# hasindu2008/squigulator

Hardware: AMD Instinct MI355X
Metric: simulated raw samples/sec (higher is better)
Workload: dtype f32+f64

## Files before the change

### squigulator_amd/csrc/h_common.h

```cpp
#pragma once

#if defined(SQG_DEV)
#define SQG_DEV_ENV(name) getenv(name)
#else
#define SQG_DEV_ENV(name) (static_cast<const char*>(nullptr))
#endif
static inline int dev_env_int(const char* v, int dflt) { return v ? atoi(v) : dflt; }

#ifndef SQG_SOURCE_HASH
#define SQG_SOURCE_HASH "unstamped"
#endif
extern "C" const char sqg_source_hash_marker[] = "SQG_SOURCE_HASH=" SQG_SOURCE_HASH ";";
#if defined(SQG_DEV)
static const char kBuildInfo[] = "source_hash=" SQG_SOURCE_HASH ";dev=1";
#else
static const char kBuildInfo[] = "source_hash=" SQG_SOURCE_HASH ";dev=0";
#endif
extern "C" const char* sqg_build_info(void) { return kBuildInfo; }

#include "h_cpus.h"

static uint32_t lcg_pow(uint32_t base, unsigned long long e) {
    uint32_t r = 1, b = base;
    while (e) { if (e & 1) r = lcg_mul(r, b); b = lcg_mul(b, b); e >>= 1; }
// ... 59 lines not shown
    DevBuf<long long> d_span; std::vector<long long> h_span;
    DevBuf<ChunkView> d_view;
    const void* span_of = nullptr; unsigned long long span_run = 0;
    void release() { *this = ChunkScratch(); }
};

struct SiteScratch {
    DevBuf<int> d_count; std::vector<int> h_count;
    DevBuf<long long> d_off; std::vector<long long> h_off;
    DevBuf<SiteRec> d_rec;
    DevBuf<uint8_t> d_skip;
    const void* plan_of = nullptr; unsigned long long plan_run = 0; int plan_key[3] = {0, 0, 0};
    void release() { *this = SiteScratch(); }
};

struct EventScratch {
    DevBuf<long long> d_start;
    DevBuf<int> d_read;
    void release() { *this = EventScratch(); }
};

struct PileupScratch {
    DevBuf<uint32_t> d_kmer;
    DevBuf<uint8_t> d_seg;
    DevBuf<PileRead> d_pr; std::vector<PileRead> h_pr;
    DevBuf<unsigned long long> d_stat;
    void release() { *this = PileupScratch(); }
};

struct DetectScratch {
    DevBuf<int> d_count; std::vector<int> h_count;
    DevBuf<long long> d_off; std::vector<long long> h_off;
    DevBuf<long long> d_start;
    DevBuf<int> d_read;
    void release() { *this = DetectScratch(); }
};

struct AlignScratch {
    DevBuf<long long> d_off;
    DevBuf<int16_t> d_level;
    DevBuf<ulonglong2> d_mask; DevBuf<int> d_lo;
    DevBuf<int> d_end;
    void release() { *this = AlignScratch(); }
};

struct sqg_ctx {
    HostPool pool_threads;
    struct DrawAhead* draw_ahead = nullptr;
    sqg_cfg_t cfg;
    int k = 0, num_kmer = 0, T = 0, wlo = 0, whi = 0, nw = 0;
    hipStream_t stream = nullptr;
    uint32_t* d_rows = nullptr;
    float2* d_model = nullptr;
    uint32_t* d_pow = nullptr;
    std::vector<uint32_t> h_pow;
    uint32_t jump2(unsigned long long n) const {
        if (n >> 32) return lcg_pow(lcg_mul(LCG_A, LCG_A), n);
        uint32_t r = h_pow[2 * POW_N + (size_t)(n & (POW_N - 1))];
        const uint32_t hi = (uint32_t)(n >> 10) & (POW_N - 1), hi2 = (uint32_t)(n >> 20);
        if (hi) r = lcg_mul(r, h_pow[3 * POW_N + hi]);
        if (hi2) r = lcg_mul(r, h_pow[4 * POW_N + hi2]);
        return r;
    }
    unsigned int* d_err = nullptr;
    unsigned long long fix_tickets = 0;
    unsigned long long scan_tickets = 0;
    struct Slot {
        int16_t* d_sig = nullptr; size_t sig_cap = 0;
        long long* d_sigoff = nullptr; size_t reads_cap = 0;
        FixEntry* d_fix = nullptr; size_t fix_cap = 0;
        unsigned int* d_fix_count = nullptr;
        FixEntry* d_fix_sh = nullptr; size_t fix_sh_cap = 0;
        unsigned int fix_sh_per = 0;
        unsigned int* d_fix_sh_count = nullptr;
        uint2* d_evrec = nullptr; size_t evrec_cap = 0;
        int* d_slow = nullptr; size_t slow_cap = 0;
        ItemDesc* d_items = nullptr; size_t items_cap = 0;
        uint32_t* d_part = nullptr; size_t part_cap = 0;
        uint32_t* d_lbase = nullptr; size_t lbase_cap = 0;
        int* d_tile_link = nullptr; size_t tile_link_cap = 0;
        uint32_t* d_part_state = nullptr; size_t part_state_cap = 0;
        hipEvent_t cal_a = nullptr, cal_b = nullptr; bool cal_pending = false; long long cal_events = 0; int cal_tries = 0; float cal_ps = 0.f;
        uint2* cal_prev = nullptr; float cal_prev_ps = 0.f;
        unsigned long long gen = 0;
        hipEvent_t done = nullptr;
        hipEvent_t sampled = nullptr;
    } slot[2];
    struct CountSet {
        uint16_t* d_dwell = nullptr; size_t dwell_cap = 0;
        uint32_t* d_tile_so = nullptr; size_t tile_cap = 0;
        unsigned long long* d_seglen = nullptr; size_t seglen_cap = 0;
        size_t seglen_dirty = 0;
        unsigned long long gen = 0;
    } cset[3];
    int num_cu = 256;
    std::deque<sqg_batch*> staged_q;
    hipStream_t fix_stream = nullptr;
    unsigned long long* d_scan_part = nullptr; size_t scan_part_cap = 0;
    uint32_t* d_link_rows = nullptr; size_t link_rows_cap = 0;
    uint32_t* d_pcnt[2] = {nullptr, nullptr}; size_t pcnt_cap[2] = {0, 0};
    uint32_t* d_slice = nullptr; size_t slice_cap = 0;
    uint32_t* d_phist = nullptr; size_t phist_cap = 0;
    double row_bound = 0;
    bool range_mode = false;
    uint32_t* d_xcounts = nullptr; size_t xcounts_cap = 0;
    struct Recycled { uint8_t* d_block; size_t block_bytes; long long* h_sigoff; long long* h_sigoff_dev; size_t h_n; hipEvent_t ev[8];
// ... 266 lines not shown
```

### squigulator_amd/csrc/h_context.h

```cpp
#pragma once

extern "C" const char* sqg_strerror(int code) {
    switch (code) {
    case SQG_OK: return "ok";
    case SQG_EINVAL: return "invalid argument or unsupported configuration";
    case SQG_ENOMEM: return "out of memory";
    case SQG_EDEVICE: return "HIP runtime error";
    case SQG_ESEQUENCE: return "batches must be run in staging order";
    case SQG_ENODEVICE: return "no usable HIP device";
    case SQG_EOVERFLOW: return "read too long (>= UINT32_MAX samples) or dwell > 65535";
    case SQG_EIO: return "file I/O error";
    default: return "unknown error";
    }
}

extern "C" const char* sqg_last_error(const sqg_ctx_t* ctx) { return ctx ? ctx->err.c_str() : ""; }

extern "C" int sqg_device_count(void) {
    int n = 0;
    if (hipGetDeviceCount(&n) != hipSuccess) return SQG_ENODEVICE;
    return n;
}

extern "C" int32_t sqg_worker_of(int32_t i, int32_t n_rec, int32_t T) {
    if (T <= 1 || n_rec <= 0) return 0;
    const int32_t step = (n_rec + T - 1) / T;
    return i / step;
}

extern "C" void sqg_destroy(sqg_ctx_t* ctx) {
    if (!ctx) return;
    if (ctx->b5_reader_drain) ctx->b5_reader_drain(ctx->b5_reader, true);
    (void)hipSetDevice(ctx->cfg.device);
    if (ctx->b5_stream) { (void)hipStreamSynchronize(ctx->b5_stream); (void)hipStreamDestroy(ctx->b5_stream); ctx->b5_stream = nullptr; }
    if (ctx->stream) (void)hipStreamSynchronize(ctx->stream);
    if (ctx->fix_stream) (void)hipStreamSynchronize(ctx->fix_stream);
    delete ctx->draw_ahead; ctx->draw_ahead = nullptr;
    (void)hipFree(ctx->d_pcnt[0]); (void)hipFree(ctx->d_pcnt[1]); (void)hipFree(ctx->d_slice); (void)hipFree(ctx->d_phist);
    (void)hipFree(ctx->d_rows); (void)hipFree(ctx->d_link_rows); (void)hipFree(ctx->d_scan_part); (void)hipFree(ctx->d_xcounts); (void)hipFree(ctx->d_model); (void)hipFree(ctx->d_samp_scratch); (void)hipFree(ctx->d_pow); (void)hipFree(ctx->d_err); (void)hipFree(ctx->d_mid_done); if (ctx->h_samp) (void)hipHostFree(ctx->h_samp);
    for (auto& Q : ctx->cset) { (void)hipFree(Q.d_dwell); (void)hipFree(Q.d_tile_so); (void)hipFree(Q.d_seglen); }
    for (auto& S : ctx->slot) {
        (void)hipFree(S.d_sig); (void)hipFree(S.d_sigoff);
        (void)hipFree(S.d_fix); (void)hipFree(S.d_fix_count); (void)hipFree(S.d_fix_sh); (void)hipFree(S.d_fix_sh_count);
        (void)hipFree(S.d_evrec); (void)hipFree(S.d_slow);
        (void)hipFree(S.d_items); (void)hipFree(S.d_part_state); (void)hipFree(S.d_part); (void)hipFree(S.d_lbase); (void)hipFree(S.d_tile_link);
        (void)hipFree(S.cal_prev);
        if (S.cal_a) (void)hipEventDestroy(S.cal_a);
        if (S.cal_b) (void)hipEventDestroy(S.cal_b);
        if (S.done) (void)hipEventDestroy(S.done);
        if (S.sampled) (void)hipEventDestroy(S.sampled);
    }
    (void)hipFree(ctx->d_svb); (void)hipFree(ctx->d_svb_size); (void)hipFree(ctx->d_svb_off);
    (void)hipFree(ctx->d_b5meta); (void)hipFree(ctx->d_b5out); (void)hipFree(ctx->d_b5tab); (void)hipFree(ctx->d_b5size); for (auto* q : ctx->h_b5out) if (q) (void)hipHostFree(q); if (ctx->h_b5meta) (void)hipHostFree(ctx->h_b5meta);
    ctx->chunk.release();
    ctx->site.release();
    ctx->event.release();
    ctx->pileup.release();
    ctx->detect.release();
    ctx->align.release();
    (void)hipFree(ctx->d_genome); (void)hipFree(ctx->d_contig_off); (void)hipFree(ctx->d_cum); (void)hipFree(ctx->d_nprefix);
    (void)hipFree(ctx->d_trans_csum); (void)hipFree(ctx->d_trans_idx); (void)hipFree(ctx->d_samp);
    (void)hipFree(ctx->d_meth); (void)hipFree(ctx->d_meth_has); (void)hipFree(ctx->d_meth_st);
    if (ctx->stage_stream) { (void)hipStreamSynchronize(ctx->stage_stream); (void)hipStreamDestroy(ctx->stage_stream); }
    for (auto& r : ctx->pool) { (void)hipFree(r.d_block); (void)hipHostFree(r.h_sigoff); (void)hipHostFree(r.h_meta); for (auto& e : r.ev) if (e) (void)hipEventDestroy(e); if (r.ev_staged) (void)hipEventDestroy(r.ev_staged); }
    ctx->pool.clear();
    if (ctx->fix_stream) (void)hipStreamDestroy(ctx->fix_stream);
    if (ctx->stream) (void)hipStreamDestroy(ctx->stream);
    delete ctx;
}

extern "C" int sqg_create(const sqg_cfg_t* cfg, sqg_ctx_t** out) {
    if (!cfg || !out) return SQG_EINVAL;
    *out = nullptr;
    if (cfg->abi_version != SQG_ABI_VERSION) return SQG_EINVAL;
    if (cfg->kmer_size < 1 || cfg->kmer_size > 9 || !cfg->model) return SQG_EINVAL;
    if (cfg->num_workers < 1 || cfg->worker_lo < 0 || cfg->worker_hi > cfg->num_workers || cfg->worker_lo >= cfg->worker_hi) return SQG_EINVAL;
    if (!(cfg->profile.range != 0.0) || !(cfg->profile.dwell_mean >= 1.0)) return SQG_EINVAL;
    if (cfg->profile.dwell_mean + 8.0 * std::fabs(cfg->profile.dwell_std) > 60000.0) return SQG_EINVAL;
    if (cfg->mode != SQG_MODE_EXACT && cfg->mode != SQG_MODE_CERTIFIED) return SQG_EINVAL;
    long long nk = 1LL << (2 * cfg->kmer_size);
    if (cfg->flags & SQG_METH) { nk = 1; for (uint32_t i = 0; i < cfg->kmer_size; i++) nk *= 5; }
    const double span = std::fabs((double)cfg->seed) + (double)cfg->num_workers * (double)(nk + 10);
    if (span > 9.0e10) return SQG_EINVAL;

    int ndev = 0;
    if (hipGetDeviceCount(&ndev) != hipSuccess || ndev <= 0) return SQG_ENODEVICE;
    if (cfg->device < 0 || cfg->device >= ndev) return SQG_EINVAL;

    sqg_ctx* c = new (std::nothrow) sqg_ctx();
    if (!c) return SQG_ENOMEM;
    c->cfg = *cfg;
    c->cfg.model = nullptr;
// ... 42 lines not shown
    CHK(hipMemset(c->d_err, 0, sizeof(unsigned int)));
    CHK(hipStreamCreateWithFlags(&c->stage_stream, hipStreamNonBlocking));
    {
        int prio_lo = 0, prio_hi = 0;
        CHK(hipDeviceGetStreamPriorityRange(&prio_lo, &prio_hi));
        CHK(hipStreamCreateWithPriority(&c->fix_stream, hipStreamNonBlocking, prio_lo));
    }
    for (auto& S : c->slot) {
        CHK(hipMalloc(&S.d_fix_count, (4 + FIX_SHARDS) * sizeof(unsigned int)));
        CHK(hipMemset(S.d_fix_count, 0, (4 + FIX_SHARDS) * sizeof(unsigned int)));
        if (cfg->mode == SQG_MODE_CERTIFIED && c->use_kmer_streams) {
            CHK(hipMalloc(&S.d_fix_sh_count, (size_t)FIX_SHARDS * FIX_SHARD_STRIDE * sizeof(unsigned int)));
            CHK(hipMemset(S.d_fix_sh_count, 0, (size_t)FIX_SHARDS * FIX_SHARD_STRIDE * sizeof(unsigned int)));
        }
        CHK(hipEventCreateWithFlags(&S.done, hipEventDisableTiming));
        CHK(hipEventCreateWithFlags(&S.sampled, hipEventDisableTiming));
        CHK(hipEventRecord(S.done, c->stream));
    }
    if (c->use_kmer_streams && !SQG_DEV_ENV("SQG_PART_CLAIMS") && !(cfg->flags & SQG_ORDER_FREE)) {
        hipDeviceProp_t prop;
        CHK(hipGetDeviceProperties(&prop, cfg->device));
        const bool listed = strncmp(prop.gcnArchName, "gfx950", 6) == 0;
        if (!listed) fprintf(stderr, "[sqg] %s is not on the list of architectures verified for lane-ordered LDS atomics: extended probe\n", prop.gcnArchName);
        unsigned int* d_bad = nullptr;
        CHK(hipMalloc(&d_bad, sizeof(unsigned int)));
        CHK(hipMemset(d_bad, 0, sizeof(unsigned int)));
        hipLaunchKernelGGL(k_lds_order_check, dim3(1024), dim3(64), 0, c->stream, listed ? 4 : 64, d_bad);
        CHK(hipGetLastError());
        unsigned int bad = 1;
        CHK(hipMemcpyAsync(&bad, d_bad, sizeof bad, hipMemcpyDeviceToHost, c->stream));
        CHK(hipStreamSynchronize(c->stream));
        (void)hipFree(d_bad);
        c->lds_ordered = bad == 0;
        if (!c->lds_ordered) fprintf(stderr, "[sqg] LDS atomics are not served in lane order on this device (%u mismatches): the claim protocol hands the k-mer streams out\n", bad);
    }
    if (cfg->mode == SQG_MODE_CERTIFIED) {
        unsigned int* d_max = nullptr;
        CHK(hipMalloc(&d_max, sizeof(unsigned int)));
        CHK(hipMemset(d_max, 0, sizeof(unsigned int)));
        hipLaunchKernelGGL(k_certify, dim3(256 * 16), dim3(256), 0, c->stream, d_max);
        CHK(hipGetLastError());
        unsigned int bits = 0;
        CHK(hipMemcpyAsync(&bits, d_max, sizeof bits, hipMemcpyDeviceToHost, c->stream));
        CHK(hipStreamSynchronize(c->stream));
        (void)hipFree(d_max);
        float m; memcpy(&m, &bits, sizeof m);
        c->delta_x_measured = m;
        if (!(m < 1.0e-4f)) { fprintf(stderr, "[sqg] certification sweep failed: max error %g\n", (double)m); return fail(SQG_EDEVICE); }
        c->delta_x = m * 1.25f + 1.0e-7f;
        if (getenv("SQG_VERBOSE")) fprintf(stderr, "[sqg] certified fp32 deviate: max |x_fp32 - x_fp64| over all states = %.3e, bound used %.3e\n", (double)m, (double)c->delta_x);
        if (const char* ov = SQG_DEV_ENV("SQG_TEST_DELTA_X")) { c->delta_x = (float)atof(ov); c->force_fix = true; }
        const double kd = cfg->profile.digitisation / cfg->profile.range;
        double lo = 1e300, hi = -1e300, eps_max = 0;
        for (long long j = 0; j < nk; j++) {
            const double mkd = (double)hm[(size_t)j].x * kd;
            const float sdk = (float)((double)hm[(size_t)j].y * kd);
            const float asdk = std::fabs(sdk);
            lo = std::min(lo, mkd - 7.0 * asdk); hi = std::max(hi, mkd + 7.0 * asdk);
            const float eps = c->delta_x * asdk + 5.9604645e-8f * ((float)std::fabs(mkd) + 21.0f * asdk + 3.0f) + 2.0e-7f;
            eps_max = std::max(eps_max, (double)eps);
        }
        c->amp_floor = lo; c->amp_ceil = hi;
        c->thr_all = std::nextafterf((float)(0.5 - eps_max * 1.000001), 0.0f);
    }
    {
        const sqg_profile_t& q = cfg->profile;
        const double a = std::floor(q.dwell_mean + 6.5556 * std::fabs(q.dwell_std) + 0.5);
        const double z = std::floor(std::fabs(q.dwell_mean - 6.5556 * std::fabs(q.dwell_std)) + 0.5) + 1.0;
        c->dwell_hi = c->use_dwell_stream ? std::max(std::max(a, z), 1.0) + 1.0 : (double)(int)q.dwell_mean;
        const double mu = std::fabs(q.dwell_mean) + 0.5, sg = c->use_dwell_stream ? std::fabs(q.dwell_std) : 0.0;
        c->lean_epl = 1;
        for (int epl = LEAN_EPL_MAX; epl >= 1; epl >>= 1) {
            const double nev = 64.0 * epl;
            if (nev * mu + 6.0 * std::sqrt(nev) * sg <= 0.97 * LEAN_MAX_SAMPLES) { c->lean_epl = epl; break; }
        }
    }

    if (c->use_kmer_streams) {
        const long long total = (long long)c->nw * nk;
        CHK(hipMalloc(&c->d_rows, (size_t)total * sizeof(uint32_t)));
        if (c->num_kmer <= 4096) {
            const int blocks = (int)((total + 255) / 256);
            hipLaunchKernelGGL(k_init_rows, dim3(blocks), dim3(256), 0, c->stream, c->d_rows, (int)nk, (long long)cfg->seed, c->wlo, total);
            CHK(hipGetLastError());
        } else {
            const char* turns_env = SQG_DEV_ENV("SQG_TEST_ROW_TURNS");
            const int turns = turns_env ? std::min(3, std::max(0, atoi(turns_env))) : 0;
            CHK(hipMemsetD32Async((hipDeviceptr_t)c->d_rows, (int)((unsigned)turns * LCG_ORD2), (size_t)total, c->stream));
            c->row_bound = (double)turns * (double)LCG_ORD2 + (turns == 3 ? (double)LCG_ORD2 : 0.0);
        }
    }
    c->time_c.resize((size_t)c->nw); c->off_x.resize((size_t)c->nw); c->med_x.resize((size_t)c->nw);
    for (int w = 0; w < c->nw; w++) {
        const long long s = (long long)cfg->seed + (long long)(w + c->wlo) * (nk + 10);
        c->time_c[(size_t)w] = canon(s + 2);
        c->off_x[(size_t)w] = s + 4;
        c->med_x[(size_t)w] = s + 5;
    }
    CHK(hipStreamSynchronize(c->stream));
#undef CHK
    *out = c;
    return SQG_OK;
}
```

### squigulator_amd/csrc/h_run.h

```cpp
#pragma once

static void count_params(sqg_ctx* c, const sqg_batch* b, sqg_ctx::CountSet& Q, const int n_part, uint32_t* d_pcnt, SigParams& P) {
    const sqg_profile_t& p = c->cfg.profile;
    P.reads = b->d_reads; P.chain_off = b->d_chain_off; P.chain_reads = b->d_chain_reads; P.chain_order = b->d_chain_order; P.bases = b->d_bases;
    P.dwell = c->use_dwell_stream ? Q.d_dwell : nullptr; P.dwell_out = Q.d_dwell; P.seglen_out = Q.d_seglen; P.seglen = Q.d_seglen; P.tile_so = Q.d_tile_so;
    P.dmean = p.dwell_mean; P.dstd = p.dwell_std; P.pw = c->d_pow; P.err = b->d_err; P.delta_x = c->delta_x;
    P.k = c->k; P.num_kmer = c->num_kmer; P.const_sps = (int)p.dwell_mean;
    P.dwell_unbounded = c->dwell_hi > 65535.0 ? 1 : 0;
    P.dwell_pack = c->dwell_hi < 1024.0 ? 1 : 0;
    P.pieces = b->d_pieces; P.piece_total = b->d_piece_total;
    P.pcnt = d_pcnt; P.n_part = n_part; P.n_links = b->n_chains;
}

struct RunStep { const char* name; std::function<int()> go; };
typedef std::vector<RunStep> RunPlan;

struct Run {
    sqg_ctx* c; sqg_batch* b; int phase; const uint32_t* before; const uint32_t* after;
    sqg_ctx::Slot* S; sqg_ctx::Slot* other; sqg_ctx::CountSet* Q;
    int n = 0, n_part = 0, dw = 0;
    bool certified = false, direct = false, fold = false, untimed = false, wave_links = false;
    size_t n_pairs = 0, n_rows = 0;
    unsigned scan_wgs = 0, pgrid = 0;
    uint32_t *d_pcnt = nullptr, *slice_lo = nullptr, *slice_hi = nullptr, *pfirst = nullptr, *pstart = nullptr, *ptotal = nullptr;
// ... 56 lines not shown
        !c->range_mode && !c->staged_q.empty() && !SQG_DEV_ENV("SQG_NO_PRECOUNT")) {
        sqg_batch* cand = c->staged_q.front();
        if (cand->seq > b->seq && cand->staged && !cand->ran && !cand->begun && !cand->precounted && cand->part && cand->pieces && cand->one == b->one &&
            cand->n > 0 && cand->n_chains > 0) {
            sqg_ctx::CountSet& NQ = c->cset[(b->run_idx + 1) % 3];
            bool ok = grow_cset(c, NQ, cand) == SQG_OK;
            const int nx = (int)((b->run_idx + 1) & 1);
            if (ok && !cand->one) ok = ensure(c, (void**)&c->d_pcnt[nx], &c->pcnt_cap[nx], (size_t)2 * cand->n_chains * (size_t)R.n_part, sizeof(uint32_t)) == SQG_OK;
            if (ok && cand->one) ok = ensure(c, (void**)&other.d_part, &other.part_cap, (size_t)cand->n_events + PART_SLACK, sizeof(uint32_t)) == SQG_OK;
            if (ok) R.pre_nb = cand;
            else c->err.clear();
        }
    }
    if (phase != 2 && b->split && !b->part && (rc = ensure(c, (void**)&c->d_link_rows, &c->link_rows_cap, (size_t)b->n_chains * (size_t)c->num_kmer, sizeof(uint32_t)))) return rc;
    if (phase != 2 && b->part) {
        if ((rc = ensure(c, (void**)&c->d_pcnt[b->run_idx & 1], &c->pcnt_cap[b->run_idx & 1], (size_t)2 * b->n_chains * (size_t)R.n_part, sizeof(uint32_t)))) return rc;
        if ((rc = ensure(c, (void**)&c->d_slice, &c->slice_cap, (size_t)2 * (size_t)b->max_slices + (size_t)3 * R.n_pairs + 1, sizeof(uint32_t)))) return rc;
        if ((rc = ensure(c, (void**)&c->d_phist, &c->phist_cap, (size_t)b->max_slices * (size_t)PART_SUB, sizeof(uint32_t)))) return rc;
    }
    if (phase == 1 && (rc = ensure(c, (void**)&c->d_xcounts, &c->xcounts_cap, R.n_rows, sizeof(uint32_t)))) return rc;
    if (n > 0 && phase != 1) {
        const size_t cap0 = c->scan_part_cap;
        if ((rc = ensure(c, (void**)&c->d_scan_part, &c->scan_part_cap, (size_t)2 * R.scan_wgs, sizeof(unsigned long long)))) return rc;
        if (c->scan_part_cap != cap0)
            HIPCHK(c, hipMemsetAsync(c->d_scan_part, 0, c->scan_part_cap * sizeof(unsigned long long), c->stream));
    }
    return SQG_OK;
}

static void run_params(Run& R) {
    sqg_ctx* c = R.c; sqg_batch* b = R.b; const int phase = R.phase, n = R.n;
    sqg_ctx::Slot& S = *R.S; sqg_ctx::CountSet& Q = *R.Q;
    const sqg_profile_t& p = c->cfg.profile;
    R.direct = c->num_kmer <= 4096;
    R.dw = c->use_dwell_stream ? (R.certified && c->dwell_hi < 1.0e6 ? 1 : 2) : 0;
    R.wave_links = b->pieces;
    const int n_part = R.n_part;
    R.d_pcnt = c->d_pcnt[b->run_idx & 1];
    R.pgrid = (unsigned)b->max_slices;
    R.slice_lo = c->d_slice;
    R.slice_hi = R.slice_lo ? R.slice_lo + (size_t)b->max_slices : nullptr;
    R.pfirst = R.slice_hi ? R.slice_hi + (size_t)b->max_slices : nullptr;
    R.pstart = R.pfirst ? R.pfirst + R.n_pairs + 1 : nullptr;
    R.ptotal = R.pstart ? R.pstart + R.n_pairs : nullptr;
    SigParams& P = R.P;
    memset(&P, 0, sizeof P);
    P.link_rows = (b->split && !b->part) ? c->d_link_rows : nullptr;
    P.part = S.d_part; P.part_state = b->part ? S.d_part_state : nullptr;
    P.poff = b->one ? b->d_link_slot : R.d_pcnt ? R.d_pcnt + (size_t)b->n_chains * n_part : nullptr;
    P.link_q = b->d_link_q;
    P.one = b->one ? 1 : 0;
    count_params(c, b, Q, n_part, R.d_pcnt, P);
    P.pstart = R.pstart;
    P.sig_off = S.d_sigoff; P.model = c->d_model; P.rows = c->d_rows;
    P.seed_base = canon((long long)c->cfg.seed + (long long)c->wlo * ((long long)c->num_kmer + 10)); P.seed_step = canon((long long)c->num_kmer + 10);
    P.dig = p.digitisation; P.range = p.range; P.kd = p.digitisation / p.range;
    P.thr_all = c->thr_all;
    P.meth = (c->cfg.flags & SQG_METH) ? 1 : 0; P.num_kmer_pad = n_part * PART_SUB;
    P.meth_top = 1; for (int i = 1; i < c->k; i++) P.meth_top *= 5u;
    P.use_streams = c->use_kmer_streams ? 1 : 0;
    P.rna = (c->cfg.flags & SQG_RNA) ? 1 : 0;
    P.evrec = S.d_evrec;
    if (b->part && b->pieces && !b->one) { P.evrec32 = reinterpret_cast<uint32_t*>(S.d_evrec); P.lbase = S.d_lbase; P.tile_link = S.d_tile_link; }
    P.tile_read = b->d_tile_read; P.stile_read = b->d_stile_read;
    const bool rna_prefix = (c->cfg.flags & SQG_RNA) && (c->cfg.flags & SQG_PREFIX);
    P.shift_len = rna_prefix ? (int)strlen(kAdaptorRna) * (int)p.dwell_mean : 0;
    {
        const double v = 30 * p.digitisation / p.range;
        int32_t t = (v > -2147483649.0 && v < 2147483648.0) ? (int32_t)v : (int32_t)0x80000000u;
        P.shift = (int)(int16_t)(uint16_t)((uint32_t)t & 0xffffu);
    }
    P.slow_count = S.d_fix_count + 1; P.items = S.d_items; P.lean_epl = c->lean_epl;
    P.slow_tiles = (R.certified && c->use_kmer_streams) ? S.d_slow : nullptr;
    R.fold = phase == 0 && n > 0 && b->n_chains > 0 && b->part && !b->one && b->pieces && R.certified && c->use_kmer_streams;
    memset(&R.SA, 0, sizeof R.SA);
    if (n > 0 && phase != 1) {
        ScanArgs& SA = R.SA;
        SA.seglen = Q.d_seglen; SA.n_reads = n; SA.sig_off = S.d_sigoff; SA.host_off = b->h_sigoff_dev; SA.err = b->d_err; SA.counters = S.d_fix_count;
        SA.part = c->d_scan_part; SA.ticket = ++c->scan_tickets; SA.shard_counters = S.d_fix_sh_count;
    }
    if (phase != 2) b->untimed = c->phase_timing_every <= 0 || (b->run_idx % c->phase_timing_every) != 0;
    R.untimed = b->untimed;
}

static void launch_events(Run& R, const int dw, const bool hist) {
    sqg_ctx* c = R.c; sqg_batch* b = R.b; const SigParams& P = R.P;
    constexpr int NT = SQG_EVENT_THREADS, NT_WIDE = 1024;
    const int wide_max = dev_env_int(SQG_DEV_ENV("SQG_EVENTS_WIDE_MAX"), 1200);
    const dim3 g((unsigned)b->n_chains);
    const bool wide = !hist && b->n_chains <= wide_max, direct = R.direct;
#define EVL(N, D, W, H, PT) hipLaunchKernelGGL((k_events<N, D, W, SQG_EVENT_EPT, H, PT>), g, dim3(N), 0, c->stream, P)
#define EVD(N, D, H, PT) do { if (dw == 0) EVL(N, D, 0, H, PT); else if (dw == 1) EVL(N, D, 1, H, PT); else EVL(N, D, 2, H, PT); } while (0)
    if (b->part) { if (hist) EVD(NT, false, true, true); else EVD(NT, false, false, true); }
    else if (wide) { if (direct) EVD(NT_WIDE, true, false, false); else EVD(NT_WIDE, false, false, false); }
    else if (direct) { if (hist) EVD(NT, true, true, false); else EVD(NT, true, false, false); }
    else { if (hist) EVD(NT, false, true, false); else EVD(NT, false, false, false); }
#undef EVD
#undef EVL
}
static void launch_part_events(Run& R, const int dwm, const bool count) {
    sqg_ctx* c = R.c; sqg_batch* b = R.b; const SigParams& P = R.P;
    if (!R.wave_links) { launch_events(R, dwm, count); return; }
    const dim3 g((unsigned)((b->n_chains + PEV_WAVES - 1) / PEV_WAVES)), t(64 * PEV_WAVES);
    if (!count) hipLaunchKernelGGL((k_part_events<0, PEV_SCATTER>), dim3((unsigned)((b->n_chains + PEV_WAVES_SCATTER - 1) / PEV_WAVES_SCATTER)), dim3(64 * PEV_WAVES_SCATTER), 0, c->stream, P, b->n_chains, (uint32_t)b->n_events);
    else if (b->one) {
        if (dwm == 0) hipLaunchKernelGGL((k_part_events<0, PEV_ONE>), g, t, 0, c->stream, P, b->n_chains, (uint32_t)b->n_events);
        else if (dwm == 1) hipLaunchKernelGGL((k_part_events<1, PEV_ONE>), g, t, 0, c->stream, P, b->n_chains, (uint32_t)b->n_events);
// ... 356 lines not shown
```

### squigulator_amd/csrc/k_common.h

```cpp
#pragma once

#define LCG_M 2147483647u
#define LCG_A 16807u

#define POW_N 1024
#define POW_TABLES 5
#define POW_TOP 4096
#define POW_WORDS (4 * POW_N + POW_TOP)
#define LCG_ORD2 1073741823u

#define NEAR_ONE_BITS 17

__host__ __device__ static inline uint32_t lcg_mul(uint32_t a, uint32_t b) {
    const unsigned long long p = (unsigned long long)a * b;
    uint32_t r = (uint32_t)(p & LCG_M) + (uint32_t)(p >> 31);
    r = (r & LCG_M) + (r >> 31);
    return r;
}
__device__ static inline uint32_t lcg_mul_lazy(uint32_t a, uint32_t b) {
    const unsigned long long p = (unsigned long long)a * b;
    return (uint32_t)(p & LCG_M) + (uint32_t)(p >> 31);
}

__device__ static inline uint32_t lcg_mul_dbl(uint32_t a, uint32_t b2) {
    const unsigned long long p2 = (unsigned long long)a * b2;
    const uint32_t r = (uint32_t)(p2 >> 32) + ((uint32_t)p2 >> 1);
    return min(r, r - LCG_M);
}

__device__ static inline uint32_t lcg_jump2(const uint32_t* __restrict__ pw, uint32_t n) {
    uint32_t r = pw[2 * POW_N + (n & (POW_N - 1))];
    const uint32_t hi = (n >> 10) & (POW_N - 1), hi2 = n >> 20;
    if (hi) r = lcg_mul(r, pw[3 * POW_N + hi]);
    if (hi2) r = lcg_mul(r, pw[4 * POW_N + hi2]);
    return r;
}

__device__ static inline double lcg_uniform(uint32_t c) {
    return (double)(c ? c : LCG_M) / 2147483647.0;
}

__device__ static inline double box_muller_exact(uint32_t c1, uint32_t c2) {
    const double u = lcg_uniform(c1);
    const double t = (2.0 * 3.14159265) * lcg_uniform(c2);
    return sqrt(-2.0 * log(u)) * cos(t);
}

__device__ static inline float box_muller_fast(uint32_t c1) {
    const float uf = (float)c1 * 4.656612873077393e-10f;
    const float lg = __builtin_amdgcn_logf(uf);
    const float y = __builtin_fmaf(lg, -1.3862943611198906f, -9.313225750491594e-10f);
    const float r = __builtin_amdgcn_sqrtf(y);
    const uint32_t plo = c1 * 16807u;
    const float t2 = __builtin_fmaf((float)(int)plo, 4.656612873077393e-10f, uf * 7.826369259425611e-06f);
    const float cs = __builtin_amdgcn_cosf(t2);
    return r * cs;
}

__device__ __attribute__((noinline)) static int dwell_exact(uint32_t c1, double dstd, double dmean) {
    const double z = box_muller_exact(c1, lcg_mul(c1, LCG_A));
    return (int)round((z * dstd) + dmean);
}

__device__ static inline int16_t to_i16(double v) {
    int32_t t;
    if (v > -2147483649.0 && v < 2147483648.0) t = (int32_t)v; else t = (int32_t)0x80000000u;
    return (int16_t)(uint16_t)((uint32_t)t & 0xffffu);
}

__device__ static inline int16_t level_code(const float2* model, uint32_t rank, double dig, double range, double offset) {
    return to_i16((double)model[rank].x * dig / range - offset);
}

__device__ static inline int16_t sample_exact(uint32_t c1, float m, float sd, double dig, double range, double offset) {
    const double z = box_muller_exact(c1, lcg_mul(c1, LCG_A));
    const float s = (float)((z * (double)sd) + (double)m);
    return to_i16((double)s * dig / range - offset);
}

// ... 36 lines not shown
    return rank;
}

struct ReadDesc {
    long long base_off;
    long long ev_off;
    double offset;
    int len0, len1;
    int ne0, ne1;
    int worker;
    uint32_t time_c0;
    int tile_off;
    int fast;
    int stile_off;
    int slot0;
};

struct FixEntry {
    long long at;
    long long ev;
    uint32_t c1;
    int read;
    int shifted;
    int pad;
};

struct ItemDesc {
    long long ev_first;
    long long sig_base;
    double offset;
    int n_ev;
    int n_samples;
    uint32_t at0;
    int ev_read0;
    int read;
    int shift_lo, shift_hi;
    int slot_first;
};

struct SigParams {
    const ReadDesc* reads;
    const int* chain_off;
    const int* chain_reads;
    const int* chain_order;
    const uint8_t* bases;
    const uint16_t* dwell;
    uint16_t* dwell_out;
    unsigned long long* seglen_out;
    int seglen_zero;
    double dmean, dstd;
    const unsigned long long* seglen;
    const long long* sig_off;
    const float2* model;
    const uint32_t* pw;
    uint32_t* rows;
    uint32_t* link_rows;
    uint32_t seed_base, seed_step;
    int16_t* sig;
    unsigned int* err;
    FixEntry* fix;
    unsigned int* fix_count;
    unsigned int fix_cap;
    FixEntry* fix_sh;
    unsigned int* fix_sh_count;
    unsigned int fix_sh_cap;
    unsigned int* fix_sh_stat;
    unsigned int* host_res;
    int fix_tag;
    uint2* evrec;
    uint32_t* evrec32;
    uint32_t* lbase;
    int* tile_link;
    uint32_t* tile_so;
    const int* tile_read;
    const int* stile_read;
    ItemDesc* items;
    int lean_epl;
    int* slow_tiles;
    unsigned int* slow_count;
    double dig, range, kd;
    float delta_x;
    float thr_all;
    int k, num_kmer;
    int meth;
    uint32_t meth_top;
    int num_kmer_pad;
    int const_sps;
    int dwell_pack;
    int dwell_unbounded;
    int use_streams;
    int rna;
    int shift_len;
    int shift;
    uint32_t* part;
    uint32_t* part_state;
    uint32_t* pcnt;
    const uint32_t* poff;
    const uint32_t* pstart;
    const int* link_q;
    int one;
    const int4* pieces;
    uint32_t* piece_total;
    int n_part;
    int n_links;
};

// ... 9 lines not shown
```

### squigulator_amd/csrc/k_samples.h

```cpp
#pragma once

struct SmpWaveLds {
    uint4 rec_a[64];
    uint2 rec_b[64];
    uint8_t mk[MK_W];
};
struct SmpLds {
    uint2 mult[MULT_N];
    SmpWaveLds w[4];
};

__device__ static inline void push_fix(const SigParams& P, bool bad, int lane, unsigned long long lane_le,
                                       long long at, uint32_t c1, long long ev, int r, int shifted) {
    const unsigned long long am = __ballot(bad);
    if (am) {
        unsigned int slot0 = 0;
        const int leader = __ffsll((long long)am) - 1;
        if (lane == leader) slot0 = atomicAdd(P.fix_count, (unsigned int)__popcll(am));
        slot0 = __shfl(slot0, leader);
        if (bad) {
            const unsigned int slot = slot0 + (unsigned int)__popcll(am & lane_le) - 1u;
            if (slot < P.fix_cap) {
                FixEntry fe; fe.at = at; fe.c1 = c1; fe.ev = ev; fe.read = r; fe.shifted = shifted; fe.pad = 0;
                P.fix[slot] = fe;
// ... 35 lines not shown
        const long long n1 = (long long)P.seglen[2 * r];
        if ((long long)base_pos + n_samples > n1 - P.shift_len && (long long)base_pos < n1) {
            shift_lo = (int)max(n1 - P.shift_len - (long long)base_pos, 0LL);
            shift_hi = (int)min(n1 - (long long)base_pos, (long long)n_samples);
        }
    }
    if (!take) {
        const int nt = (n_ev + 63) >> 6;
        const unsigned int q = atomicAdd(P.slow_count, (unsigned int)nt);
        for (int i = 0; i < nt; i++) P.slow_tiles[q + i] = rd.tile_off + lt * LEAN_EPL + i;
    }
    ItemDesc d;
    d.ev_first = rd.ev_off + (long long)lt * LEAN_EV;
    d.sig_base = sig_base;
    d.offset = rd.offset;
    d.n_ev = (take && n_samples > 0) ? n_ev : 0;
    d.n_samples = n_samples;
    d.at0 = P.rna ? read_len - 1u - base_pos : base_pos;
    d.ev_read0 = lt * LEAN_EV;
    d.read = r;
    d.shift_lo = shift_lo; d.shift_hi = shift_hi;
    d.slot_first = P.one ? rd.slot0 + lt * LEAN_EV : P.evrec32 ? (rd.slot0 >= 0 ? rd.slot0 : P.tile_link[rd.tile_off + lt * LEAN_EPL]) : 0;
    P.items[g] = d;
}
__global__ __launch_bounds__(256) void k_items(const SigParams P, const int n_stiles) { items_body(P, (int)blockIdx.x, n_stiles); }

template <typename T>
__device__ static inline T sload(const T* p) {
    static_assert(sizeof(T) % 4 == 0, "dword granularity");
    const __attribute__((address_space(4))) uint32_t* src =
        reinterpret_cast<const __attribute__((address_space(4))) uint32_t*>(reinterpret_cast<uintptr_t>(p));
    uint32_t w[sizeof(T) / 4];
#pragma unroll
    for (int q = 0; q < (int)(sizeof(T) / 4); q++) w[q] = src[q];
    T v;
    __builtin_memcpy(&v, w, sizeof v);
    return v;
}

template <int EPL>
struct LeanWaveLds {
    uint4 rec[64 * EPL];
    uint4 tb[66];
    int nfix;
    int pad[3];
    uint4 park[FIX_SLOTS];
};
template <int EPL>
struct LeanLds {
    uint32_t mult[MULT_N];
    LeanWaveLds<EPL> w[4];
};

template <bool RNA, int LEAN_EPL>
__global__ __launch_bounds__(256) void k_samples_lean(const SigParams P, const int n_stiles) {
    __shared__ LeanLds<LEAN_EPL> L;
    const int tid = threadIdx.x, lane = tid & 63;
    const int wid = __builtin_amdgcn_readfirstlane(tid >> 6);
    for (int i = tid; i < MULT_N; i += 256) L.mult[i] = P.pw[i] << 1;
    __syncthreads();
    LeanWaveLds<LEAN_EPL>& W = L.w[wid];
    const float thr = P.thr_all;
    const char* mult_b = reinterpret_cast<const char*>(L.mult);

    const unsigned xq = gridDim.x >> 3, xrem = gridDim.x & 7u, xcd = blockIdx.x & 7u;
    const unsigned wg0 = xcd * xq + min(xcd, xrem) + (blockIdx.x >> 3);
    for (int g = (int)wg0 * 4 + wid; g < n_stiles; g += gridDim.x * 4) {
        const ItemDesc it = sload(P.items + g);
        const int ne = it.n_ev;
        if (ne == 0) continue;
        const int wave_total = it.n_samples;
        const int e0 = lane * LEAN_EPL;
        const long long gev = it.ev_first + e0;
        uint2 er[LEAN_EPL];
        int sps[LEAN_EPL];
        if (P.one) {
            const uint32_t gslot = (uint32_t)it.slot_first + (uint32_t)e0;
            if (e0 + LEAN_EPL <= ne) {
                uint32_t pw_[LEAN_EPL];
                __builtin_memcpy(pw_, P.part + gslot, 4 * LEAN_EPL);
#pragma unroll
                for (int q = 0; q < LEAN_EPL; q++) { er[q] = make_uint2(gslot + (uint32_t)q, pw_[q] & 0xffffu); sps[q] = (int)(pw_[q] >> 16); }
            } else {
#pragma unroll
                for (int q = 0; q < LEAN_EPL; q++) {
                    const uint32_t w_ = e0 + q < ne ? P.part[gslot + q] : 0u;
                    er[q] = make_uint2(gslot + (uint32_t)q, w_ & 0xffffu); sps[q] = (int)(w_ >> 16);
                }
            }
        } else if (P.evrec32) {
            const uint32_t lbv = P.lbase[(size_t)it.slot_first * PART_MAX + lane];
            uint32_t ew[LEAN_EPL];
            uint16_t dw[LEAN_EPL];
            __builtin_memcpy(ew, P.evrec32 + gev, 4 * LEAN_EPL);
            if (P.dwell) __builtin_memcpy(dw, P.dwell + gev, 2 * LEAN_EPL);
            else {
#pragma unroll
                for (int q = 0; q < LEAN_EPL; q++) dw[q] = (uint16_t)P.const_sps;
            }
#pragma unroll
            for (int q = 0; q < LEAN_EPL; q++) {
                const bool v = e0 + q < ne;
                const uint32_t rank = v ? ew[q] >> EVR_REL_BITS : 0u;
                const uint32_t lb_p = (uint32_t)__builtin_amdgcn_ds_bpermute((int)((rank >> PART_SUB_BITS) << 2), (int)lbv);
                er[q] = make_uint2(v ? lb_p + (ew[q] & ((1u << EVR_REL_BITS) - 1u)) : 0u, rank);
                sps[q] = v ? (int)dw[q] : 0;
            }
        } else if (e0 + LEAN_EPL <= ne) {
            uint32_t ew[2 * LEAN_EPL];
            __builtin_memcpy(ew, P.evrec + gev, 8 * LEAN_EPL);
#pragma unroll
            for (int q = 0; q < LEAN_EPL; q++) er[q] = make_uint2(ew[2 * q], ew[2 * q + 1]);
            if (P.dwell) {
                uint16_t dw[LEAN_EPL];
                __builtin_memcpy(dw, P.dwell + gev, 2 * LEAN_EPL);
#pragma unroll
                for (int q = 0; q < LEAN_EPL; q++) sps[q] = (int)dw[q];
            } else {
#pragma unroll
                for (int q = 0; q < LEAN_EPL; q++) sps[q] = P.const_sps;
            }
        } else {
#pragma unroll
            for (int q = 0; q < LEAN_EPL; q++) {
                const bool v = e0 + q < ne;
                er[q] = v ? P.evrec[gev + q] : make_uint2(0u, 0u);
                sps[q] = v ? (P.dwell ? (int)P.dwell[gev + q] : P.const_sps) : 0;
            }
        }
        float2 md[LEAN_EPL];
#pragma unroll
        for (int q = 0; q < LEAN_EPL; q++) md[q] = (e0 + q < ne) ? P.model[er[q].y] : make_float2(0.f, 0.f);
        if (P.part_state) {
#pragma unroll
            for (int q = 0; q < LEAN_EPL; q++) if (e0 + q < ne) er[q].x = P.part_state[er[q].x];
        }
        int lane_total = 0;
#pragma unroll
        for (int q = 0; q < LEAN_EPL; q++) lane_total += sps[q];
        const int incl = wave_incl_scan_dpp(lane_total);
        __builtin_amdgcn_fence(__ATOMIC_SEQ_CST, "wavefront");
        W.tb[lane] = make_uint4(0u, 0u, 0u, 0u);
        if (lane == 0) W.nfix = 0;
        __builtin_amdgcn_fence(__ATOMIC_SEQ_CST, "wavefront");
        {
            int run = incl - lane_total;
#pragma unroll
            for (int q = 0; q < LEAN_EPL; q++) {
                const int so = run; run += sps[q];
                const double mk = (double)md[q].x * P.kd - it.offset;
                const double fl0 = floor(mk);
                const float Fh = (float)(mk - fl0 - 0.5);
                const float sdk = (float)((double)md[q].y * P.kd);
                W.rec[lane * LEAN_EPL + q] = make_uint4(er[q].x, ((uint32_t)so << 18) | ((uint32_t)(int)fl0 & 0xffffu),
                                                        __float_as_uint(Fh), __float_as_uint(sdk));
                if ((e0 + q < ne) && (lane | q) != 0) {
                    const uint32_t bit = (uint32_t)(so - 1);
                    atomicOr(reinterpret_cast<unsigned int*>(W.tb) + ((bit >> 6) << 2) + ((bit >> 5) & 1u), 1u << (bit & 31u));
                }
            }
        }
        __builtin_amdgcn_fence(__ATOMIC_SEQ_CST, "wavefront");
        {
            const uint4 mine = W.tb[lane];
            const int pc = __builtin_popcount(mine.x) + __builtin_popcount(mine.y);
            W.tb[lane].z = (uint32_t)(wave_incl_scan_dpp(pc) - pc);
        }
        __builtin_amdgcn_fence(__ATOMIC_SEQ_CST, "wavefront");
        char* const out_b = reinterpret_cast<char*>(P.sig + it.sig_base);
        uint32_t voff = RNA ? 2u * (it.at0 - (uint32_t)lane) : 2u * (it.at0 + (uint32_t)lane);
        uint32_t idx4 = (uint32_t)lane << 2;
        const int nfull = wave_total >> 6, rem = wave_total & 63;
        #define LEAN_EVOF(tq_) (int)__builtin_amdgcn_mbcnt_hi((tq_).y, __builtin_amdgcn_mbcnt_lo((tq_).x, (tq_).z))
        #define LEAN_STEP(SH, TAIL, c_, DI, ST, RA, MU, EV, RN, MN, EN, TQ, TQN) {                                       \
            EN = LEAN_EVOF(TQ);                                                                                   \
            RN = W.rec[EN];                                                                                       \
            TQN = tbp[2 + (DI)];                                                                                  \
            const uint32_t c1 = lcg_mul_dbl(RA.x, MU);                                                            \
            const float x = box_muller_fast(c1);                                                                  \
            const float vh = __builtin_fmaf(x, __uint_as_float(RA.w), __uint_as_float(RA.z));                     \
            const float t = vh + LEAN_MAGIC;                                                                      \
            const float d = vh - (t - LEAN_MAGIC);                                                                \
            const int si_ = (int)(idx4 >> 2) + 64 * (DI);                       \
            const bool act = !(TAIL) || si_ < wave_total;                                                         \
            const bool ok = fabsf(d) < thr && c1 <= LCG_M - (1u << NEAR_ONE_BITS);                                \
             \
            const bool shf = (SH) && (uint32_t)(si_ - it.shift_lo) < (uint32_t)(it.shift_hi - it.shift_lo);       \
            char* const dst_b = out_b + (RNA ? -128 * (DI) : 128 * (DI));                                         \
            if (act && ok) *reinterpret_cast<uint16_t*>(dst_b + voff) = (uint16_t)((__float_as_uint(t) + RA.y - (shf ? (uint32_t)P.shift : 0u)) & 0xffffu); \
            else if (act) {                                         \
                const unsigned long long am = __builtin_amdgcn_ballot_w64(true);                                  \
                const int n0 = W.nfix;                                                                            \
                const int slot = n0 + (int)__builtin_amdgcn_mbcnt_hi((uint32_t)(am >> 32), __builtin_amdgcn_mbcnt_lo((uint32_t)am, 0u)); \
                const uint32_t at_ = (RNA ? voff - 128u * (DI) : voff + 128u * (DI)) >> 1;                        \
                const int ev_ = EV;                                                                               \
                if (slot < FIX_SLOTS) W.park[slot] = make_uint4(at_, c1, (uint32_t)ev_, shf ? 1u : 0u);              \
                else push_fix_one(P, it.sig_base + at_, c1, it.ev_first + ev_, it.read, shf ? 1 : 0);    \
                if (slot + 1 == n0 + __popcll(am)) W.nfix = slot + 1;           \
                __builtin_amdgcn_fence(__ATOMIC_SEQ_CST, "wavefront");                                            \
            }                                                                                                     \
            if ((DI) == (ST) - 1) { idx4 += 256u * (ST); voff = RNA ? voff - 128u * (ST) : voff + 128u * (ST); tbp += (ST); } \
            MN = *reinterpret_cast<const uint32_t*>(mult_b + ((DI) == (ST) - 1 ? 0 : 256 * ((DI) + 1)) + (idx4 - (RN.y >> 16))); }
        uint4 ra, rb, tqa, tqb; uint32_t ma, mb; int eva, evb;
        const uint4* tbp = W.tb;
        {
            const uint4 tq0 = tbp[0];
            eva = LEAN_EVOF(tq0);
        }
        ra = W.rec[eva];
        tqa = tbp[1];
        ma = *reinterpret_cast<const uint32_t*>(mult_b + (idx4 - (ra.y >> 16)));
        int c = 0;
        #define LEAN_LOOP(SH)                                                                                    \
            for (; c + 4 <= nfull; c += 4) {                                                                      \
                LEAN_STEP(SH, false, c, 0, 4, ra, ma, eva, rb, mb, evb, tqa, tqb)                                 \
                LEAN_STEP(SH, false, c + 1, 1, 4, rb, mb, evb, ra, ma, eva, tqb, tqa)                             \
                LEAN_STEP(SH, false, c + 2, 2, 4, ra, ma, eva, rb, mb, evb, tqa, tqb)                             \
                LEAN_STEP(SH, false, c + 3, 3, 4, rb, mb, evb, ra, ma, eva, tqb, tqa)                             \
            }                                                                                                     \
            if (c + 2 <= nfull) {                                                                                 \
                LEAN_STEP(SH, false, c, 0, 2, ra, ma, eva, rb, mb, evb, tqa, tqb)                                 \
                LEAN_STEP(SH, false, c + 1, 1, 2, rb, mb, evb, ra, ma, eva, tqb, tqa)                             \
                c += 2;                                                                                           \
            }                                                                                                     \
            if (c < nfull) {                                                                                      \
                LEAN_STEP(SH, false, c, 0, 2, ra, ma, eva, rb, mb, evb, tqa, tqb)                                 \
                ra = rb; ma = mb; eva = evb; tqa = tqb; c++;                                                      \
                idx4 += 256u; voff = RNA ? voff - 128u : voff + 128u; tbp += 1;                                   \
            }                                                                                                     \
            if (rem) LEAN_STEP(SH, true, c, 0, 2, ra, ma, eva, rb, mb, evb, tqa, tqb)
        if (RNA && it.shift_hi > it.shift_lo) { LEAN_LOOP(true) } else { LEAN_LOOP(false) }
        #undef LEAN_LOOP
        #undef LEAN_STEP
        #undef LEAN_EVOF
        __builtin_amdgcn_fence(__ATOMIC_SEQ_CST, "wavefront");
        const int nfix = min(W.nfix, FIX_SLOTS);
        if (nfix) {
            const unsigned int sh = blockIdx.x & (FIX_SHARDS - 1);
            unsigned int at0 = 0;
            if (lane == 0) at0 = atomicAdd(P.fix_sh_count + sh * FIX_SHARD_STRIDE, (unsigned int)nfix);
            at0 = (unsigned int)__builtin_amdgcn_readfirstlane((int)at0);
            FixEntry* dst = P.fix_sh + (size_t)sh * P.fix_sh_cap + at0;
            bool room = at0 + (unsigned int)nfix <= P.fix_sh_cap;
            if (!room) {
                if (lane == 0) at0 = atomicAdd(P.fix_count, (unsigned int)nfix);
                at0 = (unsigned int)__builtin_amdgcn_readfirstlane((int)at0);
                dst = P.fix + at0;
                room = at0 + (unsigned int)nfix <= P.fix_cap;
                if (!room && lane == 0) atomicOr(P.err, 8u);
            }
            if (room && lane < nfix) {
                const uint4 pk = W.park[lane];
                FixEntry fe; fe.at = it.sig_base + pk.x; fe.c1 = pk.y; fe.ev = it.ev_first + pk.z; fe.read = it.read; fe.shifted = (int)pk.w; fe.pad = P.fix_tag;
                dst[lane] = fe;
            }
        }
    }
}

template <int MODE, bool GENERIC>
__global__ __launch_bounds__(256) void k_samples(const SigParams P, const int n_tiles) {
    __shared__ SmpLds L;
    const int tid = threadIdx.x, lane = tid & 63, wid = tid >> 6;
    for (int i = tid; i < MULT_N; i += 256) L.mult[i] = make_uint2(P.pw[i], P.pw[POW_N + i]);
    __syncthreads();
    SmpWaveLds& W = L.w[wid];
    const unsigned long long lane_le = (lane == 63) ? ~0ull : ((2ull << lane) - 1);
    const int n_work = GENERIC && P.slow_tiles ? (int)min(*P.slow_count, (unsigned int)n_tiles) : n_tiles;

    for (int wi = blockIdx.x * 4 + wid; wi < n_work; wi += gridDim.x * 4) {
        const int g = GENERIC && P.slow_tiles ? P.slow_tiles[wi] : wi;
        const int r = P.tile_read[g];
        const ReadDesc rd = P.reads[r];
        const int ne = rd.ne0 + rd.ne1;
        const int e = (g - rd.tile_off) * 64 + lane;
        const bool valid = e < ne;
        const long long ev_first = rd.ev_off + (long long)(g - rd.tile_off) * 64;
        uint2 er = make_uint2(0u, 0u);
        int sps = 0;
        if (valid) {
            if (P.one) {
                const uint32_t sl = (uint32_t)rd.slot0 + (uint32_t)e, w_ = P.part[sl];
                er = make_uint2(sl, w_ & 0xffffu);
                sps = (int)(w_ >> 16);
            } else if (P.evrec32) {
                const uint32_t w_ = P.evrec32[rd.ev_off + e], rank = w_ >> EVR_REL_BITS;
                er = make_uint2(P.lbase[(size_t)(rd.slot0 >= 0 ? rd.slot0 : P.tile_link[g]) * PART_MAX + (rank >> PART_SUB_BITS)] + (w_ & ((1u << EVR_REL_BITS) - 1u)), rank);
// ... 198 lines not shown
```

Measured before the change: 589.0 billion.

## Precompute scaled stdv table, retune LCG multiply and LDS tile-bit loads

Builds a second device model table whose y component already holds the stdv scaled by kd, computed on the host in double as before. The lean sample kernel reads it, which drops a per-event double multiply. The kernel also loads only three of the four words of each LDS tile-bit entry through an explicit address-space-3 pointer. lcg_mul_dbl is rewritten so the halving shift becomes a multiply by an opaque scalar constant, aiming at different instruction selection. These tweaks add a second model buffer and a verbose readback check, and the compiler-steering asm may not give better code.

```diff
diff --git a/squigulator_amd/csrc/h_common.h b/squigulator_amd/csrc/h_common.h
--- a/squigulator_amd/csrc/h_common.h
+++ b/squigulator_amd/csrc/h_common.h
@@ -135,6 +135,7 @@
     hipStream_t stream = nullptr;
     uint32_t* d_rows = nullptr;
     float2* d_model = nullptr;
+    float2* d_model_k = nullptr;
     uint32_t* d_pow = nullptr;
     std::vector<uint32_t> h_pow;
     uint32_t jump2(unsigned long long n) const {
diff --git a/squigulator_amd/csrc/h_context.h b/squigulator_amd/csrc/h_context.h
--- a/squigulator_amd/csrc/h_context.h
+++ b/squigulator_amd/csrc/h_context.h
@@ -37,7 +37,7 @@
     if (ctx->fix_stream) (void)hipStreamSynchronize(ctx->fix_stream);
     delete ctx->draw_ahead; ctx->draw_ahead = nullptr;
     (void)hipFree(ctx->d_pcnt[0]); (void)hipFree(ctx->d_pcnt[1]); (void)hipFree(ctx->d_slice); (void)hipFree(ctx->d_phist);
-    (void)hipFree(ctx->d_rows); (void)hipFree(ctx->d_link_rows); (void)hipFree(ctx->d_scan_part); (void)hipFree(ctx->d_xcounts); (void)hipFree(ctx->d_model); (void)hipFree(ctx->d_samp_scratch); (void)hipFree(ctx->d_pow); (void)hipFree(ctx->d_err); (void)hipFree(ctx->d_mid_done); if (ctx->h_samp) (void)hipHostFree(ctx->h_samp);
+    (void)hipFree(ctx->d_rows); (void)hipFree(ctx->d_link_rows); (void)hipFree(ctx->d_scan_part); (void)hipFree(ctx->d_xcounts); (void)hipFree(ctx->d_model); (void)hipFree(ctx->d_model_k); (void)hipFree(ctx->d_samp_scratch); (void)hipFree(ctx->d_pow); (void)hipFree(ctx->d_err); (void)hipFree(ctx->d_mid_done); if (ctx->h_samp) (void)hipHostFree(ctx->h_samp);
     for (auto& Q : ctx->cset) { (void)hipFree(Q.d_dwell); (void)hipFree(Q.d_tile_so); (void)hipFree(Q.d_seglen); }
     for (auto& S : ctx->slot) {
         (void)hipFree(S.d_sig); (void)hipFree(S.d_sigoff);
@@ -186,9 +186,11 @@
         if (const char* ov = SQG_DEV_ENV("SQG_TEST_DELTA_X")) { c->delta_x = (float)atof(ov); c->force_fix = true; }
         const double kd = cfg->profile.digitisation / cfg->profile.range;
         double lo = 1e300, hi = -1e300, eps_max = 0;
+        std::vector<float2> hk((size_t)nk);
         for (long long j = 0; j < nk; j++) {
+            hk[(size_t)j] = make_float2(hm[(size_t)j].x, (float)((double)hm[(size_t)j].y * kd));
             const double mkd = (double)hm[(size_t)j].x * kd;
-            const float sdk = (float)((double)hm[(size_t)j].y * kd);
+            const float sdk = hk[(size_t)j].y;
             const float asdk = std::fabs(sdk);
             lo = std::min(lo, mkd - 7.0 * asdk); hi = std::max(hi, mkd + 7.0 * asdk);
             const float eps = c->delta_x * asdk + 5.9604645e-8f * ((float)std::fabs(mkd) + 21.0f * asdk + 3.0f) + 2.0e-7f;
@@ -196,6 +198,23 @@
         }
         c->amp_floor = lo; c->amp_ceil = hi;
         c->thr_all = std::nextafterf((float)(0.5 - eps_max * 1.000001), 0.0f);
+        CHK(hipMalloc(&c->d_model_k, (size_t)nk * sizeof(float2)));
+        CHK(hipMemcpy(c->d_model_k, hk.data(), (size_t)nk * sizeof(float2), hipMemcpyHostToDevice));
+        if (getenv("SQG_VERBOSE")) {
+            std::vector<float2> back((size_t)nk);
+            CHK(hipMemcpy(back.data(), c->d_model_k, (size_t)nk * sizeof(float2), hipMemcpyDeviceToHost));
+            long long differ = 0;
+            unsigned long long sum = 0;
+            for (long long j = 0; j < nk; j++) {
+                const float sd = cfg->model[j].level_stdv * cfg->amp_noise;
+                const float want = (float)((double)sd * kd);
+                uint32_t bw, bg, bm0, bm1;
+                memcpy(&bw, &want, 4); memcpy(&bg, &back[(size_t)j].y, 4); memcpy(&bm0, &cfg->model[j].level_mean, 4); memcpy(&bm1, &back[(size_t)j].x, 4);
+                differ += (bw != bg) || (bm0 != bm1);
+                sum += (unsigned long long)bg * (unsigned long long)(j + 1);
+            }
+            fprintf(stderr, "[sqg] model_k: %lld rows read back from the device, %lld differ from {level_mean, (float)((double)stdv * kd)}, sdk bits sum %llu\n", nk, differ, sum);
+        }
     }
     {
         const sqg_profile_t& q = cfg->profile;
diff --git a/squigulator_amd/csrc/h_run.h b/squigulator_amd/csrc/h_run.h
--- a/squigulator_amd/csrc/h_run.h
+++ b/squigulator_amd/csrc/h_run.h
@@ -132,7 +132,7 @@
     P.one = b->one ? 1 : 0;
     count_params(c, b, Q, n_part, R.d_pcnt, P);
     P.pstart = R.pstart;
-    P.sig_off = S.d_sigoff; P.model = c->d_model; P.rows = c->d_rows;
+    P.sig_off = S.d_sigoff; P.model = c->d_model; P.model_k = c->d_model_k; P.rows = c->d_rows;
     P.seed_base = canon((long long)c->cfg.seed + (long long)c->wlo * ((long long)c->num_kmer + 10)); P.seed_step = canon((long long)c->num_kmer + 10);
     P.dig = p.digitisation; P.range = p.range; P.kd = p.digitisation / p.range;
     P.thr_all = c->thr_all;
diff --git a/squigulator_amd/csrc/k_common.h b/squigulator_amd/csrc/k_common.h
--- a/squigulator_amd/csrc/k_common.h
+++ b/squigulator_amd/csrc/k_common.h
@@ -23,8 +23,10 @@
 }
 
 __device__ static inline uint32_t lcg_mul_dbl(uint32_t a, uint32_t b2) {
+    uint32_t half = 0x80000000u;
+    asm("" : "+s"(half));
     const unsigned long long p2 = (unsigned long long)a * b2;
-    const uint32_t r = (uint32_t)(p2 >> 32) + ((uint32_t)p2 >> 1);
+    const uint32_t r = (uint32_t)(((unsigned long long)(uint32_t)p2 * half + p2) >> 32);
     return min(r, r - LCG_M);
 }
 
@@ -167,6 +169,7 @@
     const unsigned long long* seglen;
     const long long* sig_off;
     const float2* model;
+    const float2* model_k;
     const uint32_t* pw;
     uint32_t* rows;
     uint32_t* link_rows;
diff --git a/squigulator_amd/csrc/k_samples.h b/squigulator_amd/csrc/k_samples.h
--- a/squigulator_amd/csrc/k_samples.h
+++ b/squigulator_amd/csrc/k_samples.h
@@ -111,6 +111,10 @@
     LeanWaveLds<EPL> w[4];
 };
 
+struct alignas(16) __attribute__((may_alias)) LeanTbEntry { uint32_t x, y, z, w; };
+typedef const __attribute__((address_space(3))) LeanTbEntry* lean_tb_ptr;
+__device__ static inline uint4 lean_tb_ld(lean_tb_ptr p) { return make_uint4(p->x, p->y, p->z, 0u); }
+
 template <bool RNA, int LEAN_EPL>
 __global__ __launch_bounds__(256) void k_samples_lean(const SigParams P, const int n_stiles) {
     __shared__ LeanLds<LEAN_EPL> L;
@@ -189,7 +193,7 @@
         }
         float2 md[LEAN_EPL];
 #pragma unroll
-        for (int q = 0; q < LEAN_EPL; q++) md[q] = (e0 + q < ne) ? P.model[er[q].y] : make_float2(0.f, 0.f);
+        for (int q = 0; q < LEAN_EPL; q++) md[q] = (e0 + q < ne) ? P.model_k[er[q].y] : make_float2(0.f, 0.f);
         if (P.part_state) {
 #pragma unroll
             for (int q = 0; q < LEAN_EPL; q++) if (e0 + q < ne) er[q].x = P.part_state[er[q].x];
@@ -210,7 +214,7 @@
                 const double mk = (double)md[q].x * P.kd - it.offset;
                 const double fl0 = floor(mk);
                 const float Fh = (float)(mk - fl0 - 0.5);
-                const float sdk = (float)((double)md[q].y * P.kd);
+                const float sdk = md[q].y;
                 W.rec[lane * LEAN_EPL + q] = make_uint4(er[q].x, ((uint32_t)so << 18) | ((uint32_t)(int)fl0 & 0xffffu),
                                                         __float_as_uint(Fh), __float_as_uint(sdk));
                 if ((e0 + q < ne) && (lane | q) != 0) {
@@ -230,11 +234,12 @@
         uint32_t voff = RNA ? 2u * (it.at0 - (uint32_t)lane) : 2u * (it.at0 + (uint32_t)lane);
         uint32_t idx4 = (uint32_t)lane << 2;
         const int nfull = wave_total >> 6, rem = wave_total & 63;
+        #define LEAN_TB(i_) lean_tb_ld(tbp + (i_))
         #define LEAN_EVOF(tq_) (int)__builtin_amdgcn_mbcnt_hi((tq_).y, __builtin_amdgcn_mbcnt_lo((tq_).x, (tq_).z))
         #define LEAN_STEP(SH, TAIL, c_, DI, ST, RA, MU, EV, RN, MN, EN, TQ, TQN) {                                       \
             EN = LEAN_EVOF(TQ);                                                                                   \
             RN = W.rec[EN];                                                                                       \
-            TQN = tbp[2 + (DI)];                                                                                  \
+            TQN = LEAN_TB(2 + (DI));                                                                             \
             const uint32_t c1 = lcg_mul_dbl(RA.x, MU);                                                            \
             const float x = box_muller_fast(c1);                                                                  \
             const float vh = __builtin_fmaf(x, __uint_as_float(RA.w), __uint_as_float(RA.z));                     \
@@ -261,13 +266,15 @@
             if ((DI) == (ST) - 1) { idx4 += 256u * (ST); voff = RNA ? voff - 128u * (ST) : voff + 128u * (ST); tbp += (ST); } \
             MN = *reinterpret_cast<const uint32_t*>(mult_b + ((DI) == (ST) - 1 ? 0 : 256 * ((DI) + 1)) + (idx4 - (RN.y >> 16))); }
         uint4 ra, rb, tqa, tqb; uint32_t ma, mb; int eva, evb;
-        const uint4* tbp = W.tb;
+        uint32_t tb_addr = (uint32_t)reinterpret_cast<uintptr_t>((lean_tb_ptr)reinterpret_cast<const LeanTbEntry*>(W.tb));
+        if (!RNA) asm("" : "+v"(tb_addr));
+        lean_tb_ptr tbp = reinterpret_cast<lean_tb_ptr>((uintptr_t)tb_addr);
         {
-            const uint4 tq0 = tbp[0];
+            const uint4 tq0 = LEAN_TB(0);
             eva = LEAN_EVOF(tq0);
         }
         ra = W.rec[eva];
-        tqa = tbp[1];
+        tqa = LEAN_TB(1);
         ma = *reinterpret_cast<const uint32_t*>(mult_b + (idx4 - (ra.y >> 16)));
         int c = 0;
         #define LEAN_LOOP(SH)                                                                                    \
@@ -292,6 +299,7 @@
         #undef LEAN_LOOP
         #undef LEAN_STEP
         #undef LEAN_EVOF
+        #undef LEAN_TB
         __builtin_amdgcn_fence(__ATOMIC_SEQ_CST, "wavefront");
         const int nfix = min(W.nfix, FIX_SLOTS);
         if (nfix) {
```

Result: no change. 591.8 billion, median of 6 (+0.5%).
